# rg2/DeepFluoroLabeling-IPCAI2020

Hardware: AMD Instinct MI355X
Metric: train images/sec, paper U-Net (depth 6, wf 5, BN, strided-conv down, seg + 14-landmark heads), 1x192x192 (8x-downsampled 184x184 padded) (higher is better)
Workload: dtype bf16 (bf16 activations, activation gradients and GEMM weight copies in HBM; bf16 MFMA, fp32 accumulate, BatchNorm statistics, losses, weight gradients and master weights); 1 GPU; BASELINE configs[1]: 8x-downsampled, seg + 14-landmark heat-map dual head, batch 16 per GPU, Dice+NCC loss, SGD nesterov; global_batch=16, image=1x192x192, parallelism=dp1, math=bf16s, optimizer=dfl_amd.SGD(momentum 0.9, nesterov, wd 1e-4)

## Files before the change

deepfluorolabeling-ipcai2020_amd/csrc/convp.h:

```cpp
#pragma once
#include "common.h"

namespace dfl {

struct ConvP {
  dfl_conv_args a;
  int Mtot, Cout;
  int Hg, Wg;
  int PH, PW, IPP;
  int npy, npx, npatch;
  int IH, IW;
  int CK, nblk, blk_per_slice;
  int splits, T;
  int pix_stride, upp_shift;
  int lds_bytes, tile;
  int ntiles, grid, xcd_mode;
  uint32_t x_bytes, w_bytes;
  uint32_t x2_bytes, xo_bytes;
  uint32_t mPP, mPW;
  int tab_off, pad1;
  int s_mt, s_nt, s_ksplit_shift, s_cpk_shift, s_ksteps, s_kper;
  uint32_t qm_npatch, qm_ntiles, qm_perimg, qm_npx;
  int q_ngroups, q_stride;
};
constexpr int CONVS_TILE = 39;
constexpr int CONVQ_TILE = 40;
constexpr int CONVQ_LAYOUTS = 9;
constexpr int CONVN_TILE = 58;
constexpr int CONVN_LAYOUTS = 6;
constexpr int CONVN_PERS_TILE = 64;

int convp_plan(const dfl_conv_args* a, ConvP* p, int force_splits);
int convp_launch(const ConvP& p, hipStream_t s);
int convp_finish_rows(const ConvP& p);
int convp_candidates(const dfl_conv_args* a, int32_t* out, int max);
int convp_force(const int32_t* g);
int convp_tune_add(const int32_t* key, const int32_t* g);

bool convq_shape_ok(const dfl_conv_args& a);
int convq_launch(const ConvP& p, int mode, int pers, hipStream_t s);
size_t convq_lds_bytes(int ck, int mode, int blk_per_slice, int pers);
int convq_threads(int mode);
bool convq_pers_ok(int mode, int ck, int x_mode);
bool convq_ck_ok(int mode, int ck);

bool convn_shape_ok(const dfl_conv_args& a);
bool convn_layout_ok(int layout, int ntot, int cin);
void convn_patch(int layout, int* ph, int* pw);
size_t convn_lds_bytes(int layout, int cin, int ntot, int pers);
bool convn_pers_ok(int layout, const dfl_conv_args& a);
int convn_launch(const ConvP& p, int layout, int pers, hipStream_t s);

bool convs_eligible(const dfl_conv_args& a, const ConvP& p);
void convs_plan(const dfl_conv_args& a, ConvP* p, int force_splits);
int convs_launch(const ConvP& p, hipStream_t s);
bool convs_first_ok(const dfl_conv_args* a);
int convs_first_launch(const dfl_conv_args* a, hipStream_t s);
int convs_pair_ok(const dfl_conv_args* a, const dfl_conv_args* b);
int convs_pair_launch(const dfl_conv_args* a, const dfl_conv_args* b, hipStream_t s);

bool convs32_eligible(const dfl_conv_args* a);
int convs32_suggest_splits(const dfl_conv_args* a);
int convs32_launch(const dfl_conv_args* a, hipStream_t s, int* splits_out);
int convs32_pair_ok(const dfl_conv_args* a, const dfl_conv_args* b);
int convs32_pair_launch(const dfl_conv_args* a, const dfl_conv_args* b, hipStream_t s);

struct WgP;
int wgradp_suggest_splits(const dfl_wgrad_args* a);
int wgradp_launch(const dfl_wgrad_args* a, hipStream_t s);
int wgradp_config(const dfl_wgrad_args* a);

}
```

deepfluorolabeling-ipcai2020_amd/csrc/wgradp_bf16.hip:

```cpp
#include <stdlib.h>
#include <string.h>

#include <mutex>
#include <vector>

#include "common.h"
#include "convp.h"

namespace dfl {

constexpr uint32_t WPOOB = 0x80000000u;
typedef unsigned int wpu32x4 __attribute__((ext_vector_type(4)));
typedef short ws16x4_t __attribute__((ext_vector_type(4)));

struct WgP {
  dfl_wgrad_args a;
  int Mtot, T;
  int PH, PW, IPP, npy, npx, npatch;
  int IH, IW;
  int P16;
  int CMT, CGT;
  int pairs, phases;
  int zslices, patches_per_slice;
  int sd, sg;
  int dupp_shift, gupp_shift;
  int g_off;
  int tab_off;
  int lds_bytes;
  long long* trace;
  uint32_t g_bytes, d_bytes;
  uint32_t d2_bytes;
  int xcd_map;
};

__device__ __forceinline__ float wbf_lo(uint32_t w) { return __uint_as_float(w << 16); }
__device__ __forceinline__ float wbf_hi(uint32_t w) { return __uint_as_float(w & 0xffff0000u); }
__device__ __forceinline__ uint32_t wpack_bf2(float a, float b) {
  const bf16x2_t h = __builtin_convertvector((f32x2_t){a, b}, bf16x2_t);
  return __builtin_bit_cast(uint32_t, h);
}

__device__ __forceinline__ bf16x8_t wtr_read8(const unsigned char* base, uint32_t r0, uint32_t r1) {
  typedef __attribute__((address_space(3))) ws16x4_t* lds_p;
  const ws16x4_t x = __builtin_amdgcn_ds_read_tr16_b64_v4i16((lds_p)(base + r0));
  const ws16x4_t y = __builtin_amdgcn_ds_read_tr16_b64_v4i16((lds_p)(base + r1));
  return __builtin_bit_cast(bf16x8_t, __builtin_shufflevector(x, y, 0, 1, 2, 3, 4, 5, 6, 7));
}

typedef unsigned int wpu32x2 __attribute__((ext_vector_type(2)));
__device__ __forceinline__ wpu32x2 wtr_read4(const unsigned char* base, uint32_t r0) {
  typedef __attribute__((address_space(3))) ws16x4_t* lds_p;
  return __builtin_bit_cast(wpu32x2, __builtin_amdgcn_ds_read_tr16_b64_v4i16((lds_p)(base + r0)));
}

__host__ __device__ constexpr int wgp_max_d_units(int KH, bool dbrb = false) { return KH == 3 ? (dbrb ? 1536 : 2304) : 1024; }
__host__ __device__ constexpr int wgp_max_g_units(int KH, bool dbrb = false) { return KH == 3 ? (dbrb ? 3072 : 4608) : 2048; }

template <int KH, int KW, bool AFF, bool DBRB = false, bool BIAS = DBRB>
__global__ void __launch_bounds__(256 * KH, KH == 2 ? 4 : 3) wgradp_kernel(const WgP p) {
  constexpr int NT = 256 * KH;
  constexpr int T = KH * KW;
  extern __shared__ __attribute__((aligned(16))) unsigned char smem[];
  const dfl_wgrad_args& a = p.a;
#ifdef DFL_WGP_TRACE
  const long long tr_entry = __builtin_amdgcn_s_memtime();
#endif
  const int tid = threadIdx.x, lane = tid & 63, wave = tid >> 6;
  const int li = lane & 31, lh = lane >> 5;
  const int ty = wave % KH, slot = wave / KH;
  const int pair = slot % p.pairs, phase = slot / p.pairs;
  const int pairs_n = p.CGT >> 5;
  const int pm = pair / pairs_n, pn = pair - pm * pairs_n;
  int bx = blockIdx.x, by = blockIdx.y, bz = blockIdx.z;
  if (p.xcd_map) {
    const int gx = gridDim.x, gy = gridDim.y, nt = gx * gy;
    const int total = nt * (int)gridDim.z, per = total >> 3;
    const int L = bx + gx * (by + gy * bz);
    const int Lp = L < (per << 3) ? (L & 7) * per + (L >> 3) : L;
    bz = Lp / nt;
    const int t = Lp - bz * nt;
    bx = t / gy;
    by = t - bx * gy;
  }
  const int cm0 = bx * p.CMT, cg0 = by * p.CGT;
  unsigned char* Ds = smem;
  unsigned char* Gs = smem + p.g_off;

  __amdgpu_buffer_rsrc_t rsD = __builtin_amdgcn_make_buffer_rsrc(const_cast<float*>(a.d), 0, (int)p.d_bytes, 0x00020000);
  __amdgpu_buffer_rsrc_t rsG = __builtin_amdgcn_make_buffer_rsrc(const_cast<float*>(a.g), 0, (int)p.g_bytes, 0x00020000);
  __amdgpu_buffer_rsrc_t rsD2 = rsD;
  if constexpr (DBRB) rsD2 = __builtin_amdgcn_make_buffer_rsrc(const_cast<float*>(a.d2), 0, (int)p.d2_bytes, 0x00020000);

  f32x16 acc[KW];
#pragma unroll
  for (int t = 0; t < KW; ++t)
#pragma unroll
    for (int r = 0; r < 16; ++r) acc[t][r] = 0.f;

  const int trow = 8 * lh + ((lane & 15) >> 2);
  const uint32_t tcb = (uint32_t)((16 * ((lane >> 4) & 1) + 4 * (lane & 3)) * 2);
  const uint32_t d_col = (uint32_t)(pm * 64) + tcb, g_col = (uint32_t)(pn * 64) + tcb;

  const int dupp = p.CMT >> 3, gupp = p.CGT >> 3;
  const int npix_g = p.IPP * p.IH * p.IW;
  const int per_img = p.npy * p.npx;
  uint32_t* gtab = reinterpret_cast<uint32_t*>(smem + p.tab_off);

  constexpr int MAXD = wgp_max_d_units(KH, DBRB) / NT, MAXG = wgp_max_g_units(KH, DBRB) / NT;
  wpu32x4 dreg[MAXD], greg[MAXG];
  wpu32x4 d2reg[DBRB ? MAXD : 1];
  float bsum = 0.f;
  const bool bias_on = BIAS && a.bias_partial != nullptr && by == 0;
  uint32_t dpos[MAXD], gpos[MAXG];
  uint32_t gok = 0;
  const int ddk = NT >> p.dupp_shift, gdk = NT >> p.gupp_shift;
  const int dcq = tid & (dupp - 1), gcq = tid & (gupp - 1);
  const int dc = cm0 + dcq * 8, gc = cg0 + gcq * 8;
  const uint32_t dpitch = (uint32_t)a.ldd * 2u, gpitch = (uint32_t)a.ldg * 2u, d2pitch = (uint32_t)a.ldd2 * 2u;
  const int nd = (p.P16 * dupp + NT - 1) / NT, ng = (npix_g * gupp + NT - 1) / NT;
  {
    const int PHW = p.PH * p.PW;
#pragma unroll
    for (int u = 0; u < MAXD; ++u) {
      const int k = (tid >> p.dupp_shift) + u * ddk;
      const int img = k / PHW, r = k - img * PHW;
      const int y = r / p.PW, x = r - y * p.PW;
      const bool live = k < p.P16 && img < p.IPP && dc < a.Cm;
      dpos[u] = (uint32_t)y | ((uint32_t)x << 12) | ((uint32_t)(img & 127) << 24) | (live ? 0x80000000u : 0u);
    }
    const int IHW = p.IH * p.IW;
#pragma unroll
    for (int u = 0; u < MAXG; ++u) {
      const int k = (tid >> p.gupp_shift) + u * gdk;
      const int img = k / IHW, r = k - img * IHW;
      const int y = r / p.IW, x = r - y * p.IW;
      const bool live = k < npix_g && gc < a.Cg;
      gpos[u] = (uint32_t)y | ((uint32_t)x << 12) | ((uint32_t)(img & 127) << 24) | (live ? 0x80000000u : 0u);
    }
    for (int j = tid; j < p.P16; j += NT) {
      const int img = j / PHW, r = j - img * PHW;
      const int y = r / p.PW, x = r - y * p.PW;
      gtab[j] = img < p.IPP ? (uint32_t)((img * p.IH + y * a.stride) * p.IW + x * a.stride) * (uint32_t)p.sg : 0u;
    }
  }
  float* aff = reinterpret_cast<float*>(smem + p.tab_off + p.P16 * 4);
  float* dco = aff + 2 * p.CGT;
  int is_nleft = 0, is_oy0 = 0, is_ox0 = 0, is_ybase = 0, is_xbase = 0;
  uint32_t is_dbase = 0, is_dbase2 = 0, is_gbase = 0;
  auto issue_setup = [&](int patch, bool live) {
    const int pg = patch / per_img, pr = patch - pg * per_img;
    const int ppy = pr / p.npx, ppx = pr - ppy * p.npx;
    const int img0 = pg * p.IPP;
    is_oy0 = ppy * p.PH;
    is_ox0 = ppx * p.PW;
    is_nleft = live ? a.N - img0 : 0;
    is_dbase = (uint32_t)(((img0 * a.Hout + is_oy0) * a.Wout + is_ox0) * a.ldd + dc) * 2u;
    is_dbase2 = DBRB ? (uint32_t)(((img0 * a.Hout + is_oy0) * a.Wout + is_ox0) * a.ldd2 + dc) * 2u : 0u;
    is_ybase = is_oy0 * a.stride - a.pad;
    is_xbase = is_ox0 * a.stride - a.pad;
    is_gbase = (uint32_t)(((img0 * a.Hin + is_ybase) * a.Win + is_xbase) * a.ldg + gc) * 2u;
    gok = 0;
  };
  auto issue_d = [&](int u) {
    if (u < nd) {
      const uint32_t q = dpos[u];
      const int qy = (int)(q & 0xfffu), qx = (int)((q >> 12) & 0xfffu), qi = (int)((q >> 24) & 127u);
      const bool ok = (int)q < 0 && qi < is_nleft && is_oy0 + qy < a.Hout && is_ox0 + qx < a.Wout;
      const uint32_t rel = (uint32_t)((qi * a.Hout + qy) * a.Wout + qx) * dpitch;
      dreg[u] = __builtin_amdgcn_raw_buffer_load_b128(rsD, ok ? is_dbase + rel : WPOOB, 0, 0);
      if constexpr (DBRB) {
        const uint32_t rel2 = (uint32_t)((qi * a.Hout + qy) * a.Wout + qx) * d2pitch;
        d2reg[u] = __builtin_amdgcn_raw_buffer_load_b128(rsD2, ok ? is_dbase2 + rel2 : WPOOB, 0, 0);
      }
    }
  };
  auto issue_g = [&](int u) {
    if (u < ng) {
      const uint32_t q = gpos[u];
      const int qy = (int)(q & 0xfffu), qx = (int)((q >> 12) & 0xfffu), qi = (int)((q >> 24) & 127u);
      const bool ok = (int)q < 0 && qi < is_nleft && (unsigned)(is_ybase + qy) < (unsigned)a.Hin && (unsigned)(is_xbase + qx) < (unsigned)a.Win;
      gok |= ok ? (1u << u) : 0u;
      const uint32_t rel = (uint32_t)((qi * a.Hin + qy) * a.Win + qx) * gpitch;
      greg[u] = __builtin_amdgcn_raw_buffer_load_b128(rsG, ok ? is_gbase + rel : WPOOB, 0, 0);
    }
  };
  auto issue = [&](int patch, bool live) {
    issue_setup(patch, live);
#pragma unroll
    for (int u = 0; u < MAXD; ++u) issue_d(u);
#pragma unroll
    for (int u = 0; u < MAXG; ++u) issue_g(u);
  };
  auto commit = [&]() {
#pragma unroll
    for (int u = 0; u < MAXD; ++u) {
      const int k = (tid >> p.dupp_shift) + u * ddk;
      if (u < nd && k < p.P16) {
        wpu32x4 v = dreg[u];
        if constexpr (DBRB) {
          const wpu32x4 r = d2reg[u];
          const float4 a0 = *reinterpret_cast<const float4*>(dco + dcq * 8), a1 = *reinterpret_cast<const float4*>(dco + dcq * 8 + 4);
          const float4 b0 = *reinterpret_cast<const float4*>(dco + p.CMT + dcq * 8), b1 = *reinterpret_cast<const float4*>(dco + p.CMT + dcq * 8 + 4);
          const float4 c0 = *reinterpret_cast<const float4*>(dco + 2 * p.CMT + dcq * 8), c1 = *reinterpret_cast<const float4*>(dco + 2 * p.CMT + dcq * 8 + 4);
          auto brb = [](float dy, float rv, float A, float B, float Cc) { return rv > 0.f ? fmaf(A, dy, fmaf(B, rv, Cc)) : 0.f; };
          v.x = wpack_bf2(brb(wbf_lo(v.x), wbf_lo(r.x), a0.x, b0.x, c0.x), brb(wbf_hi(v.x), wbf_hi(r.x), a0.y, b0.y, c0.y));
          v.y = wpack_bf2(brb(wbf_lo(v.y), wbf_lo(r.y), a0.z, b0.z, c0.z), brb(wbf_hi(v.y), wbf_hi(r.y), a0.w, b0.w, c0.w));
          v.z = wpack_bf2(brb(wbf_lo(v.z), wbf_lo(r.z), a1.x, b1.x, c1.x), brb(wbf_hi(v.z), wbf_hi(r.z), a1.y, b1.y, c1.y));
          v.w = wpack_bf2(brb(wbf_lo(v.w), wbf_lo(r.w), a1.z, b1.z, c1.z), brb(wbf_hi(v.w), wbf_hi(r.w), a1.w, b1.w, c1.w));
        }
        *reinterpret_cast<wpu32x4*>(Ds + (uint32_t)k * (uint32_t)p.sd + (uint32_t)dcq * 16u) = v;
      }
    }
#pragma unroll
    for (int u = 0; u < MAXG; ++u) {
      const int pix = (tid >> p.gupp_shift) + u * gdk;
      if (u < ng && pix < npix_g) {
        wpu32x4 v = greg[u];
        if constexpr (AFF) {
          if ((gok >> u) & 1u) {
            const float4 s0 = *reinterpret_cast<const float4*>(aff + gcq * 8), s1 = *reinterpret_cast<const float4*>(aff + gcq * 8 + 4);
            const float4 h0 = *reinterpret_cast<const float4*>(aff + p.CGT + gcq * 8), h1 = *reinterpret_cast<const float4*>(aff + p.CGT + gcq * 8 + 4);
            const float sc[8] = {s0.x, s0.y, s0.z, s0.w, s1.x, s1.y, s1.z, s1.w}, sh[8] = {h0.x, h0.y, h0.z, h0.w, h1.x, h1.y, h1.z, h1.w};
            v.x = wpack_bf2(fmaf(wbf_lo(v.x), sc[0], sh[0]), fmaf(wbf_hi(v.x), sc[1], sh[1]));
            v.y = wpack_bf2(fmaf(wbf_lo(v.y), sc[2], sh[2]), fmaf(wbf_hi(v.y), sc[3], sh[3]));
            v.z = wpack_bf2(fmaf(wbf_lo(v.z), sc[4], sh[4]), fmaf(wbf_hi(v.z), sc[5], sh[5]));
            v.w = wpack_bf2(fmaf(wbf_lo(v.w), sc[6], sh[6]), fmaf(wbf_hi(v.w), sc[7], sh[7]));
          }
        }
        *reinterpret_cast<wpu32x4*>(Gs + (uint32_t)pix * (uint32_t)p.sg + (uint32_t)gcq * 16u) = v;
      }
    }
  };

  const int pbegin = bz * p.patches_per_slice;
  const int pend = min(pbegin + p.patches_per_slice, p.npatch);
  const int nsteps = p.P16 >> 4;
  const uint32_t gadd = g_col + (uint32_t)(ty * p.IW) * (uint32_t)p.sg;
  const uint32_t dstep = (uint32_t)(16 * p.phases) * (uint32_t)p.sd;
  const bool al8 = KW == 3 && a.stride == 1 && (p.PW & 7) == 0;
#ifdef DFL_WGP_TRACE
  long long tr[8] = {0, 0, 0, 0, 0, 0, 0, 0};
  tr[0] = __builtin_amdgcn_s_memtime();
  tr[6] = __builtin_amdgcn_s_memrealtime();
#define WTR(i, t0) tr[i] += __builtin_amdgcn_s_memtime() - (t0);
#define WT0(name) const long long name = __builtin_amdgcn_s_memtime();
#else
#define WTR(i, t0)
#define WT0(name)
#endif
  issue(pbegin, pbegin < pend);
  if constexpr (AFF) {
    for (int c = tid; c < p.CGT; c += NT) {
      aff[c] = (cg0 + c < a.Cg) ? a.in_scale[cg0 + c] : 1.f;
      aff[p.CGT + c] = (cg0 + c < a.Cg) ? a.in_shift[cg0 + c] : 0.f;
    }
  }
  if constexpr (DBRB) {
    for (int c = tid; c < p.CMT; c += NT) {
      const bool live = a.coef != nullptr && cm0 + c < a.Cm;
      float A = live ? a.coef[cm0 + c] : 1.f, B = live ? a.coef[a.Cm + cm0 + c] : 0.f, Cc = live ? a.coef[2 * a.Cm + cm0 + c] : 0.f;
      if (a.coef_tot != nullptr && cm0 + c < a.Cm)
        bn_live_coef(a.coef_tot, a.bn_gamma, a.bn_mean, a.bn_invstd, a.bn_count, a.Cm, cm0 + c, &A, &B, &Cc);
      dco[c] = A;
      dco[p.CMT + c] = B;
      dco[2 * p.CMT + c] = Cc;
    }
  }
  if constexpr (AFF || DBRB) __syncthreads();
  for (int patch = pbegin; patch < pend; ++patch) {
    WT0(tb0)
    if (patch != pbegin) __syncthreads();
    WTR(1, tb0)
    WT0(tc0)
    commit();
    WTR(2, tc0)
    WT0(tb1)
    __syncthreads();
    WTR(1, tb1)
    WT0(ti0)
    issue(patch + 1, patch + 1 < pend);
    WTR(3, ti0)
    if constexpr (BIAS) {
      if (bias_on) {
        const int bc = tid & (p.CMT - 1), bstride = NT / p.CMT;
        for (int r = tid / p.CMT; r < p.P16; r += bstride)
          bsum += __uint_as_float((uint32_t)*reinterpret_cast<const unsigned short*>(Ds + (uint32_t)r * (uint32_t)p.sd + (uint32_t)bc * 2u) << 16);
      }
    }
    WT0(tk0)
    uint32_t dr0 = (uint32_t)(phase * 16 + trow) * (uint32_t)p.sd + d_col;
    const uint32_t* tp = gtab + phase * 16 + trow;
    int ks = phase;
    auto kstep = [&]() {
      const uint32_t gr0 = tp[0] + gadd, gr1 = tp[4] + gadd;
      const bf16x8_t df = wtr_read8(Ds, dr0, dr0 + 4u * (uint32_t)p.sd);
      bf16x8_t gf[KW];
      if (KW == 3 && al8) {
        const wpu32x2 g0 = wtr_read4(Gs, gr0), g1 = wtr_read4(Gs, gr1), g2 = wtr_read4(Gs, gr0 + 8u * (uint32_t)p.sg);
        gf[0] = __builtin_bit_cast(bf16x8_t, (wpu32x4){g0.x, g0.y, g1.x, g1.y});
        gf[1] = __builtin_bit_cast(bf16x8_t, (wpu32x4){__builtin_amdgcn_alignbit(g0.y, g0.x, 16), __builtin_amdgcn_alignbit(g1.x, g0.y, 16),
                                                        __builtin_amdgcn_alignbit(g1.y, g1.x, 16), __builtin_amdgcn_alignbit(g2.x, g1.y, 16)});
        gf[KW - 1] = __builtin_bit_cast(bf16x8_t, (wpu32x4){g0.y, g1.x, g1.y, g2.x});
      } else {
#pragma unroll
        for (int t = 0; t < KW; ++t) gf[t] = wtr_read8(Gs, gr0 + (uint32_t)(t * p.sg), gr1 + (uint32_t)(t * p.sg));
      }
#pragma unroll
      for (int t = 0; t < KW; ++t) acc[t] = __builtin_amdgcn_mfma_f32_32x32x16_bf16(df, gf[t], acc[t], 0, 0, 0);
      dr0 += dstep;
      tp += 16 * p.phases;
      ks += p.phases;
    };
    while (ks < nsteps) kstep();
    WTR(4, tk0)
  }
#ifdef DFL_WGP_TRACE
  tr[5] = __builtin_amdgcn_s_memtime();
#endif

  if constexpr (BIAS) {
    if (a.bias_partial != nullptr && by == 0) {
      __syncthreads();
      float* bred = reinterpret_cast<float*>(smem);
      bred[tid] = bsum;
      __syncthreads();
      for (int c = tid; c < p.CMT; c += NT) {
        float t = 0.f;
        for (int th = c; th < NT; th += p.CMT) t += bred[th];
        if (cm0 + c < a.Cm) a.bias_partial[(int64_t)bz * a.Cm + cm0 + c] = t;
      }
    }
  }

  if (p.phases > 1) {
    float* red = reinterpret_cast<float*>(smem);
#pragma unroll
    for (int t = 0; t < KW; ++t) {
      __syncthreads();
      if (phase > 0) {
        float* dst = red + ((((phase - 1) * p.pairs + pair) * KH + ty) * 16) * 64 + lane;
#pragma unroll
        for (int r = 0; r < 16; ++r) dst[r * 64] = acc[t][r];
      }
      __syncthreads();
      if (phase == 0) {
        for (int ph = 1; ph < p.phases; ++ph) {
          const float* src = red + ((((ph - 1) * p.pairs + pair) * KH + ty) * 16) * 64 + lane;
#pragma unroll
          for (int r = 0; r < 16; ++r) acc[t][r] += src[r * 64];
        }
      }
    }
    if (phase > 0 && p.zslices > 1) return;
  }
#ifdef DFL_WGP_TRACE
  const long long tr_main_end = __builtin_amdgcn_s_memtime();
#endif
  const bool sliced = p.zslices > 1;
  const int cgl = pn * 32 + li, cg = cg0 + cgl;
  if (sliced) {
    float* out = a.partial + (int64_t)bz * a.Cm * a.Cg * T;
#pragma unroll
    for (int tx = 0; tx < KW; ++tx) {
      const int t = ty * KW + tx;
#pragma unroll
      for (int r = 0; r < 16; ++r) {
        const int cm = cm0 + pm * 32 + mfma32_row(r, lane);
        if (cm < a.Cm && cg < a.Cg) out[((int64_t)t * a.Cm + cm) * a.Cg + cg] = acc[tx][r];
      }
    }
  } else {
    __syncthreads();
    float* tile = reinterpret_cast<float*>(smem);
    if (phase == 0) {
#pragma unroll
      for (int tx = 0; tx < KW; ++tx) {
        const int t = ty * KW + tx;
#pragma unroll
        for (int r = 0; r < 16; ++r) tile[((pm * 32 + mfma32_row(r, lane)) * p.CGT + cgl) * T + t] = acc[tx][r];
      }
    }
    __syncthreads();
    const int row4 = p.CGT * T / 4;
    const int valid4 = min(p.CGT, a.Cg - cg0) * T / 4;
    for (int idx = tid; idx < p.CMT * row4; idx += NT) {
      const int row = idx / row4, c4 = idx - row * row4;
      if (cm0 + row < a.Cm && c4 < valid4)
        *reinterpret_cast<float4*>(a.dw + ((int64_t)(cm0 + row) * a.Cg + cg0) * T + c4 * 4) = *reinterpret_cast<const float4*>(tile + (row * p.CGT) * T + c4 * 4);
    }
  }
#ifdef DFL_WGP_TRACE
  __builtin_amdgcn_s_waitcnt(0);
  if (tid == 0 && p.trace != nullptr) {
    long long* sink = p.trace + (int64_t)(blockIdx.x + gridDim.x * (blockIdx.y + gridDim.y * blockIdx.z)) * 12;
    for (int i = 0; i < 6; ++i) sink[i] = tr[i];
    sink[6] = tr_main_end;
    sink[7] = tr[6];
    sink[8] = __builtin_amdgcn_s_memrealtime();
    sink[10] = tr_entry;
    sink[11] = __builtin_amdgcn_s_memtime();
    sink[9] = 1;
  }
#endif
}


static int pitch_for(int channels) {
  const int data = channels * 2;
  int pitch = data;
  while (pitch % 256 != 64 && pitch % 256 != 192) pitch += 16;
  return pitch;
}

static int wgp_plan(const dfl_wgrad_args* a, WgP* p, bool need_out) {
  DFL_REQUIRE(a != nullptr, "dfl_conv2d_wgrad: null args");
  DFL_REQUIRE(a->N > 0 && a->Hin > 0 && a->Win > 0 && a->Cg > 0 && a->Cm > 0, "dfl_conv2d_wgrad: bad sizes");
  DFL_REQUIRE(a->KH > 0 && a->KW > 0 && a->stride > 0 && a->pad >= 0, "dfl_conv2d_wgrad: bad window");
  const int T = a->KH * a->KW;
  DFL_REQUIRE((a->KH == 1 && a->KW == 1) || (a->KH == 2 && a->KW == 2) || (a->KH == 3 && a->KW == 3),
              "dfl_conv2d_wgrad (bf16): 1x1, 2x2 and 3x3 windows");
  const int ho = (a->Hin + 2 * a->pad - a->KH) / a->stride + 1;
  const int wo = (a->Win + 2 * a->pad - a->KW) / a->stride + 1;
  DFL_REQUIRE(ho == a->Hout && wo == a->Wout, "dfl_conv2d_wgrad: Hout/Wout (%d,%d) do not match the window (%d,%d)", a->Hout,
              a->Wout, ho, wo);
  DFL_REQUIRE(a->Cg % 8 == 0 && a->Cm % 8 == 0 && a->ldg % 8 == 0 && a->ldd % 8 == 0 && aligned16(a->g) && aligned16(a->d),
              "dfl_conv2d_wgrad (bf16): channel counts and pixel strides must be multiples of 8, tensors 16-byte aligned");
  DFL_REQUIRE((a->in_scale == nullptr) == (a->in_shift == nullptr), "dfl_conv2d_wgrad: in_scale/in_shift go together");
  if (need_out) {
    DFL_REQUIRE(a->g && a->d, "dfl_conv2d_wgrad: g and d are required");
    DFL_REQUIRE(a->splits >= 1, "dfl_conv2d_wgrad: splits >= 1");
    DFL_REQUIRE(a->splits > 1 ? a->partial != nullptr : a->dw != nullptr, "dfl_conv2d_wgrad: output buffer missing");
  }
  memset(p, 0, sizeof(*p));
  p->a = *a;
  p->T = T;
  const int64_t M = (int64_t)a->N * a->Hout * a->Wout;
  DFL_REQUIRE(M < (1ll << 31), "dfl_conv2d_wgrad: too many pixels");
  p->Mtot = (int)M;
  const int64_t gb = (((int64_t)a->N * a->Hin * a->Win - 1) * a->ldg + a->Cg) * 2;
  const int64_t db = ((M - 1) * a->ldd + a->Cm) * 2;
  const int64_t lim = (1ll << 31) - 4096;
  DFL_REQUIRE(gb < lim && db < lim, "dfl_conv2d_wgrad (bf16): tensors must stay below 2 GiB");
  p->g_bytes = (uint32_t)gb;
  p->d_bytes = (uint32_t)db;
  if (a->d_mode != 0) {
    DFL_REQUIRE(a->coef_tot == nullptr || (a->coef == nullptr && a->bn_gamma && a->bn_mean && a->bn_invstd && a->bn_count > 0),
                "dfl_conv2d_wgrad (bf16): coef_tot replaces coef and needs bn_gamma, bn_mean, bn_invstd, bn_count");
    DFL_REQUIRE(a->d_mode == 1 && a->KH == 3 && a->d2 != nullptr && a->ldd2 % 8 == 0 && aligned16(a->d2),
                "dfl_conv2d_wgrad (bf16): d_mode 1 needs a 3x3 window and d2 (16-byte aligned, ldd2 %% 8 == 0)");
    const int64_t d2b = ((M - 1) * a->ldd2 + a->Cm) * 2;
    DFL_REQUIRE(d2b < lim, "dfl_conv2d_wgrad (bf16): tensors must stay below 2 GiB");
    p->d2_bytes = (uint32_t)d2b;
  }
  DFL_REQUIRE(a->bias_partial == nullptr || a->KH == 3, "dfl_conv2d_wgrad (bf16): bias_partial is implemented by the 3x3 kernel");
  p->CMT = a->Cm > 32 ? 64 : 32;
  p->CGT = a->Cg > 32 ? 64 : 32;
  {
    static const int small_from = [] {
      const char* e = getenv("DFL_WGP_SMALL_TILES");
      return e ? atoi(e) : 4;
    }();
    constexpr int small_from21 = 4;
    const int64_t tiles64 = ceil_div(a->Cm, 64) * ceil_div(a->Cg, 64);
    const int from = a->KH == 3 ? small_from : small_from21;
    if (from > 0 && a->Cm > 32 && a->Cg > 32 && tiles64 >= from && tiles64 < 256) p->CMT = p->CGT = 32;
  }
  p->pairs = (p->CMT / 32) * (p->CGT / 32);
  p->phases = 4 / p->pairs;
  p->dupp_shift = p->CMT == 64 ? 3 : 2;
  p->gupp_shift = p->CGT == 64 ? 3 : 2;
  p->sd = pitch_for(p->CMT);
  p->sg = pitch_for(p->CGT);
  const int64_t max_du = wgp_max_d_units(a->KH, a->d_mode != 0), max_gu = wgp_max_g_units(a->KH, a->d_mode != 0);
  const int lds_cap = a->KH == 3 ? 120 * 1024 : (a->KH == 2 ? 72 * 1024 : 52 * 1024);
  auto geom = [&](int ipp_, int ph_, int pw_, int64_t* lds, int64_t* du, int64_t* gu) {
    const int p16 = (ipp_ * ph_ * pw_ + 15) / 16 * 16;
    const int ih = (ph_ - 1) * a->stride + a->KH, iw = (pw_ - 1) * a->stride + a->KW;
    *du = (int64_t)p16 * (p->CMT / 8);
    *gu = (int64_t)ipp_ * ih * iw * (p->CGT / 8);
    *lds = (int64_t)p16 * p->sd + (int64_t)ipp_ * ih * iw * p->sg + (int64_t)p16 * 4 + 512;
  };
  auto fits = [&](int ipp_, int ph_, int pw_) {
    int64_t lds, du, gu;
    geom(ipp_, ph_, pw_, &lds, &du, &gu);
    return lds <= lds_cap && du <= max_du && gu <= max_gu && ipp_ <= 127 && ph_ < 4096 && pw_ < 4096;
  };
  int ipp = 0, ph = 0, pw = 0;
  double best_cost = 1e300;
  struct PatchMemo { int key[8]; int ipp, ph, pw; };
  static std::mutex memo_mu;
  static std::vector<PatchMemo> memo;
  const int mkey[8] = {a->N, a->Hout, a->Wout, a->stride, a->KH + 16 * (a->d_mode != 0 ? 1 : 0), a->KW, p->CMT, p->CGT};
  bool found = false;
  {
    std::lock_guard<std::mutex> lock(memo_mu);
    for (const PatchMemo& m : memo)
      if (memcmp(m.key, mkey, sizeof(mkey)) == 0) {
        ipp = m.ipp; ph = m.ph; pw = m.pw;
        found = true;
        break;
      }
  }
  auto consider = [&](int ipp_, int ph_, int pw_) {
    if (ipp_ < 1 || ph_ < 1 || pw_ < 1 || ph_ > a->Hout || pw_ > a->Wout || !fits(ipp_, ph_, pw_)) return;
    int64_t lds, du, gu;
    geom(ipp_, ph_, pw_, &lds, &du, &gu);
    const double npatch = (double)ceil_div(a->N, ipp_) * (double)ceil_div(a->Hout, ph_) * (double)ceil_div(a->Wout, pw_);
    constexpr double charge = 24.0 * 1024.0;
    double cost = npatch * ((double)(du + gu) * 16.0 + charge);
    if (a->KH == 3 && a->stride == 1 && pw_ % 8 == 0) cost *= 0.92;
    if (cost < best_cost) {
      best_cost = cost;
      ipp = ipp_;
      ph = ph_;
      pw = pw_;
    }
  };
  if (!found) {
    for (int n = a->N; n >= 1; --n) consider(n, a->Hout, a->Wout);
    for (int pw_ = 4; pw_ <= a->Wout; ++pw_) {
      if (pw_ != a->Wout && pw_ % 4 != 0) continue;
      for (int ph_ = 1; ph_ <= a->Hout; ++ph_) {
        if (!fits(1, ph_, pw_)) break;
        consider(1, ph_, pw_);
      }
    }
    if (ipp == 0) consider(1, 1, a->Wout < 4 ? a->Wout : 4);
    DFL_REQUIRE(ipp > 0, "dfl_conv2d_wgrad (bf16): no patch of this layer fits the staging limits");
    PatchMemo m;
    memcpy(m.key, mkey, sizeof(mkey));
    m.ipp = ipp; m.ph = ph; m.pw = pw;
    std::lock_guard<std::mutex> lock(memo_mu);
    if (memo.size() < 4096) memo.push_back(m);
  }
  p->IPP = ipp;
  p->PH = ph;
  p->PW = pw;
  p->P16 = (ipp * ph * pw + 15) / 16 * 16;
  p->npy = (int)ceil_div(a->Hout, ph);
  p->npx = (int)ceil_div(a->Wout, pw);
  p->npatch = (int)ceil_div(a->N, ipp) * p->npy * p->npx;
  p->IH = (ph - 1) * a->stride + a->KH;
  p->IW = (pw - 1) * a->stride + a->KW;
  p->g_off = (p->P16 * p->sd + 255) / 256 * 256;
  p->tab_off = (p->g_off + (ipp * p->IH * p->IW + 2) * p->sg + 255) / 256 * 256;
  p->lds_bytes = p->tab_off + p->P16 * 4 + 2 * p->CGT * 4 + 3 * p->CMT * 4;
  if ((a->d_mode != 0 || a->bias_partial != nullptr) && p->lds_bytes < 256 * a->KH * 4) p->lds_bytes = 256 * a->KH * 4;
  const int red_bytes = (p->phases - 1) * p->pairs * a->KH * 16 * 64 * 4;
  if (p->lds_bytes < red_bytes) p->lds_bytes = red_bytes;
  return DFL_OK;
}

static int wgp_slices(const WgP& p) {
  const int64_t tiles = ceil_div(p.a.Cm, p.CMT) * ceil_div(p.a.Cg, p.CGT);
  constexpr int target3 = 256;
  constexpr int target21 = 512;
  const int target = p.a.KH == 3 ? target3 : target21;
  int64_t z = ceil_div(target, tiles);
  if (z > p.npatch) z = p.npatch;
  if (z < 1) z = 1;
  const int64_t pps = ceil_div(p.npatch, z);
  z = ceil_div(p.npatch, pps);
  return (int)z;
}

int wgradp_suggest_splits(const dfl_wgrad_args* a) {
  WgP p;
  int rc = wgp_plan(a, &p, false);
  if (rc != DFL_OK) return rc;
  return wgp_slices(p);
}

int wgradp_config(const dfl_wgrad_args* a) {
  WgP p;
  int rc = wgp_plan(a, &p, false);
  if (rc != DFL_OK) return rc;
  return 16 + (p.T == 9 ? 0 : (p.T == 4 ? 1 : 2));
}

template <int KH, int KW>
static int wgp_launch_t(const WgP& p_in, hipStream_t s) {
  WgP p = p_in;
  dim3 grid((unsigned)ceil_div(p.a.Cm, p.CMT), (unsigned)ceil_div(p.a.Cg, p.CGT), (unsigned)p.zslices);
  p.xcd_map = (grid.x * grid.y > 1 && grid.x * grid.y * grid.z >= 16) ? 1 : 0;
  const size_t lds = (size_t)p.lds_bytes;
#define DFL_WGP_LAUNCH(AFF_, DBRB_, BIAS_)                                                                                       \
  {                                                                                                                              \
    auto k = wgradp_kernel<KH, KW, AFF_, DBRB_, BIAS_>;                                                                          \
    DFL_LDS_OPT_IN(k, 150 * 1024, "dfl_conv2d_wgrad (bf16)") \
    hipLaunchKernelGGL(k, grid, dim3(256 * KH), lds, s, p);                                                                      \
  }
  const bool aff = p.a.in_scale != nullptr;
  if constexpr (KH == 3) {
    if (p.a.d_mode != 0) {
      if (aff) DFL_WGP_LAUNCH(true, true, true) else DFL_WGP_LAUNCH(false, true, true)
      return check_launch("dfl_conv2d_wgrad (bf16)");
    }
    if (p.a.bias_partial != nullptr) {
      if (aff) DFL_WGP_LAUNCH(true, false, true) else DFL_WGP_LAUNCH(false, false, true)
      return check_launch("dfl_conv2d_wgrad (bf16)");
    }
  }
  if (aff) DFL_WGP_LAUNCH(true, false, false) else DFL_WGP_LAUNCH(false, false, false)
#undef DFL_WGP_LAUNCH
  return check_launch("dfl_conv2d_wgrad (bf16)");
}

int wgradp_launch(const dfl_wgrad_args* a, hipStream_t s) {
  WgP p;
  int rc = wgp_plan(a, &p, true);
  if (rc != DFL_OK) return rc;
  p.zslices = a->splits;
  p.patches_per_slice = (int)ceil_div(p.npatch, p.zslices);
  if (p.zslices == 1 && p.lds_bytes < p.CMT * p.CGT * p.T * 4) p.lds_bytes = p.CMT * p.CGT * p.T * 4;
#ifdef DFL_WGP_TRACE
  {
    const char* e = getenv("DFL_WGP_TRACE_PTR");
    p.trace = e ? reinterpret_cast<long long*>(strtoull(e, nullptr, 0)) : nullptr;
    fprintf(stderr, "wgradp: tile %dx%d pairs %d phases %d patch %dx%dx%d (P16 %d) gathered %dx%d slices %d patches/slice %d lds %d\n", p.CMT, p.CGT, p.pairs,
            p.phases, p.IPP, p.PH, p.PW, p.P16, p.IH, p.IW, p.zslices, p.patches_per_slice, p.lds_bytes);
  }
#endif
  switch (p.T) {
    case 9: return wgp_launch_t<3, 3>(p, s);
    case 4: return wgp_launch_t<2, 2>(p, s);
    default: return wgp_launch_t<1, 1>(p, s);
  }
}

}
```

Measured before the change: 4523 images/sec.

## Add row-streaming 3x3 weight-gradient kernel with rolling input-row ring in LDS

```diff
diff --git a/deepfluorolabeling-ipcai2020_amd/csrc/convp.h b/deepfluorolabeling-ipcai2020_amd/csrc/convp.h
--- a/deepfluorolabeling-ipcai2020_amd/csrc/convp.h
+++ b/deepfluorolabeling-ipcai2020_amd/csrc/convp.h
@@ -69,5 +69,8 @@
 int wgradp_suggest_splits(const dfl_wgrad_args* a);
 int wgradp_launch(const dfl_wgrad_args* a, hipStream_t s);
 int wgradp_config(const dfl_wgrad_args* a);
+bool wgradn_applies(const dfl_wgrad_args* a);
+int wgradn_suggest_splits(const dfl_wgrad_args* a);
+int wgradn_launch(const dfl_wgrad_args* a, hipStream_t s);
 
 }
diff --git a/deepfluorolabeling-ipcai2020_amd/csrc/wgradn_bf16.hip b/deepfluorolabeling-ipcai2020_amd/csrc/wgradn_bf16.hip
--- /dev/null
+++ b/deepfluorolabeling-ipcai2020_amd/csrc/wgradn_bf16.hip
@@ -0,0 +1,448 @@
+#include <stdlib.h>
+#include <string.h>
+
+#include <algorithm>
+
+#include "common.h"
+#include "convp.h"
+
+namespace dfl {
+
+namespace {
+
+constexpr uint32_t WNOOB = 0x80000000u;
+constexpr int WN_NT = 512;
+typedef unsigned int wnu32x4 __attribute__((ext_vector_type(4)));
+typedef unsigned int wnu32x2 __attribute__((ext_vector_type(2)));
+typedef short wns16x4_t __attribute__((ext_vector_type(4)));
+
+template <bool DBRB> struct WnUnits { static constexpr int D = DBRB ? 2 : 3, G = 4; };
+
+struct WgN {
+  dfl_wgrad_args a;
+  int Hg;
+  int Vtot;
+  int PH, W16, GW, RG;
+  int CMT, CGT, pairs, phases;
+  int ncg, nb, RB;
+  int zslices, rows_per_slice;
+  int sd, sg;
+  int g_off, tab_off, lds_bytes;
+  uint32_t g_bytes, d_bytes, d2_bytes;
+};
+
+__device__ __forceinline__ float wn_lo(uint32_t w) { return __uint_as_float(w << 16); }
+__device__ __forceinline__ float wn_hi(uint32_t w) { return __uint_as_float(w & 0xffff0000u); }
+__device__ __forceinline__ uint32_t wn_pack(float a, float b) {
+  const bf16x2_t h = __builtin_convertvector((f32x2_t){a, b}, bf16x2_t);
+  return __builtin_bit_cast(uint32_t, h);
+}
+__device__ __forceinline__ wnu32x2 wn_tr4(const unsigned char* base, uint32_t off) {
+  typedef __attribute__((address_space(3))) wns16x4_t* lds_p;
+  return __builtin_bit_cast(wnu32x2, __builtin_amdgcn_ds_read_tr16_b64_v4i16((lds_p)(base + off)));
+}
+
+template <bool AFF, bool DBRB, bool BIAS>
+__global__ void __launch_bounds__(WN_NT, 2) wgradn_kernel(const WgN p) {
+  constexpr int NT = WN_NT;
+  constexpr int MAXD = WnUnits<DBRB>::D, MAXG = WnUnits<DBRB>::G;
+  extern __shared__ __attribute__((aligned(16))) unsigned char smem[];
+  const dfl_wgrad_args& a = p.a;
+  const int tid = threadIdx.x, lane = tid & 63, wave = tid >> 6;
+  const int pair = wave % p.pairs, phase = wave / p.pairs;
+  const int pairs_n = p.CGT >> 5;
+  const int pm = pair / pairs_n, pn = pair - pm * pairs_n;
+  const int bz = blockIdx.z;
+  const int cm0 = blockIdx.x * p.CMT, cg0 = blockIdx.y * p.CGT;
+  unsigned char* Ds = smem;
+  unsigned char* Gs = smem + p.g_off;
+  float* aff = reinterpret_cast<float*>(smem + p.tab_off);
+  float* dco = aff + 2 * p.CGT;
+
+  __amdgpu_buffer_rsrc_t rsD = __builtin_amdgcn_make_buffer_rsrc(const_cast<float*>(a.d), 0, (int)p.d_bytes, 0x00020000);
+  __amdgpu_buffer_rsrc_t rsG = __builtin_amdgcn_make_buffer_rsrc(const_cast<float*>(a.g), 0, (int)p.g_bytes, 0x00020000);
+  __amdgpu_buffer_rsrc_t rsD2 = rsD;
+  if constexpr (DBRB) rsD2 = __builtin_amdgcn_make_buffer_rsrc(const_cast<float*>(a.d2), 0, (int)p.d2_bytes, 0x00020000);
+
+  const int dupp = p.CMT >> 3, gupp = p.CGT >> 3;
+  const int dcq = tid & (dupp - 1), gcq = tid & (gupp - 1);
+  const int dk0 = tid / dupp, dks = NT / dupp, gk0 = tid / gupp, gks = NT / gupp;
+  const int dc = cm0 + dcq * 8, gc = cg0 + gcq * 8;
+  const int dpix = p.PH * p.W16, gpix = p.PH * p.GW;
+  const uint32_t dpitch = (uint32_t)a.ldd * 2u, gpitch = (uint32_t)a.ldg * 2u, d2pitch = (uint32_t)a.ldd2 * 2u;
+  uint32_t dpos[MAXD], gpos[MAXG];
+#pragma unroll
+  for (int u = 0; u < MAXD; ++u) {
+    const int k = dk0 + u * dks, y = k / p.W16, x = k - y * p.W16;
+    dpos[u] = (k < dpix && x < a.Wout && dc < a.Cm) ? ((uint32_t)y | ((uint32_t)x << 16)) : 0xffffffffu;
+  }
+#pragma unroll
+  for (int u = 0; u < MAXG; ++u) {
+    const int k = gk0 + u * gks, y = k / p.GW, x = k - y * p.GW;
+    const int ix = x - a.pad;
+    gpos[u] = (k < gpix && ix >= 0 && ix < a.Win && gc < a.Cg) ? ((uint32_t)y | ((uint32_t)x << 16)) : 0xffffffffu;
+  }
+  wnu32x4 dreg[MAXD], greg[MAXG];
+  wnu32x4 d2reg[DBRB ? MAXD : 1];
+  uint32_t gok = 0;
+  int is_gslot = 0;
+
+  const int v0 = bz * p.rows_per_slice;
+  const int v1 = min(v0 + p.rows_per_slice, p.Vtot);
+  auto issue = [&](int pi) {
+    const int vb = v0 + pi * p.PH;
+    if (pi >= 0) {
+      const int img0 = vb / p.Hg, oy0 = vb - img0 * p.Hg;
+#pragma unroll
+      for (int u = 0; u < MAXD; ++u) {
+        const uint32_t q = dpos[u];
+        const int y = (int)(q & 0xffffu), x = (int)(q >> 16);
+        int oy = oy0 + y, img = img0;
+        if (oy >= p.Hg) { oy -= p.Hg; ++img; }
+        const bool ok = q != 0xffffffffu && vb + y < v1 && oy < a.Hout && img < a.N;
+        const uint32_t row = (uint32_t)(img * a.Hout + oy) * (uint32_t)a.Wout + (uint32_t)x;
+        dreg[u] = __builtin_amdgcn_raw_buffer_load_b128(rsD, ok ? row * dpitch + (uint32_t)dc * 2u : WNOOB, 0, 0);
+        if constexpr (DBRB) d2reg[u] = __builtin_amdgcn_raw_buffer_load_b128(rsD2, ok ? row * d2pitch + (uint32_t)dc * 2u : WNOOB, 0, 0);
+      }
+    }
+    const int Y0 = vb + 2;
+    const int Yc = Y0 < 0 ? 0 : Y0;
+    const int img0 = Yc / p.Hg, y0 = Yc - img0 * p.Hg;
+    is_gslot = ((Y0 % p.RG) + p.RG) % p.RG;
+    gok = 0;
+#pragma unroll
+    for (int u = 0; u < MAXG; ++u) {
+      const uint32_t q = gpos[u];
+      const int y = (int)(q & 0xffffu), x = (int)(q >> 16);
+      int yy = y0 + y + (Y0 < 0 ? Y0 : 0), img = img0;
+      if (yy >= p.Hg) { yy -= p.Hg; ++img; }
+      const int iy = yy - a.pad;
+      const bool ok = q != 0xffffffffu && Y0 + y >= 0 && iy >= 0 && iy < a.Hin && img < a.N;
+      gok |= ok ? (1u << u) : 0u;
+      const uint32_t pix = (uint32_t)(img * a.Hin + iy) * (uint32_t)a.Win + (uint32_t)(x - a.pad);
+      greg[u] = __builtin_amdgcn_raw_buffer_load_b128(rsG, ok ? pix * gpitch + (uint32_t)gc * 2u : WNOOB, 0, 0);
+    }
+  };
+  auto commit = [&](bool with_d) {
+    if (with_d) {
+#pragma unroll
+      for (int u = 0; u < MAXD; ++u) {
+        const int k = dk0 + u * dks;
+        if (k < dpix) {
+          wnu32x4 v = dreg[u];
+          if constexpr (DBRB) {
+            const wnu32x4 r = d2reg[u];
+            const float4 a0 = *reinterpret_cast<const float4*>(dco + dcq * 8), a1 = *reinterpret_cast<const float4*>(dco + dcq * 8 + 4);
+            const float4 b0 = *reinterpret_cast<const float4*>(dco + p.CMT + dcq * 8), b1 = *reinterpret_cast<const float4*>(dco + p.CMT + dcq * 8 + 4);
+            const float4 c0 = *reinterpret_cast<const float4*>(dco + 2 * p.CMT + dcq * 8), c1 = *reinterpret_cast<const float4*>(dco + 2 * p.CMT + dcq * 8 + 4);
+            auto brb = [](float dy, float rv, float A, float B, float Cc) { return rv > 0.f ? fmaf(A, dy, fmaf(B, rv, Cc)) : 0.f; };
+            v.x = wn_pack(brb(wn_lo(v.x), wn_lo(r.x), a0.x, b0.x, c0.x), brb(wn_hi(v.x), wn_hi(r.x), a0.y, b0.y, c0.y));
+            v.y = wn_pack(brb(wn_lo(v.y), wn_lo(r.y), a0.z, b0.z, c0.z), brb(wn_hi(v.y), wn_hi(r.y), a0.w, b0.w, c0.w));
+            v.z = wn_pack(brb(wn_lo(v.z), wn_lo(r.z), a1.x, b1.x, c1.x), brb(wn_hi(v.z), wn_hi(r.z), a1.y, b1.y, c1.y));
+            v.w = wn_pack(brb(wn_lo(v.w), wn_lo(r.w), a1.z, b1.z, c1.z), brb(wn_hi(v.w), wn_hi(r.w), a1.w, b1.w, c1.w));
+          }
+          *reinterpret_cast<wnu32x4*>(Ds + (uint32_t)k * (uint32_t)p.sd + (uint32_t)dcq * 16u) = v;
+        }
+      }
+    }
+#pragma unroll
+    for (int u = 0; u < MAXG; ++u) {
+      const int k = gk0 + u * gks;
+      if (k < gpix) {
+        const int y = k / p.GW, x = k - y * p.GW;
+        int slot = is_gslot + y;
+        if (slot >= p.RG) slot -= p.RG;
+        wnu32x4 v = greg[u];
+        if constexpr (AFF) {
+          if ((gok >> u) & 1u) {
+            const float4 s0 = *reinterpret_cast<const float4*>(aff + gcq * 8), s1 = *reinterpret_cast<const float4*>(aff + gcq * 8 + 4);
+            const float4 h0 = *reinterpret_cast<const float4*>(aff + p.CGT + gcq * 8), h1 = *reinterpret_cast<const float4*>(aff + p.CGT + gcq * 8 + 4);
+            v.x = wn_pack(fmaf(wn_lo(v.x), s0.x, h0.x), fmaf(wn_hi(v.x), s0.y, h0.y));
+            v.y = wn_pack(fmaf(wn_lo(v.y), s0.z, h0.z), fmaf(wn_hi(v.y), s0.w, h0.w));
+            v.z = wn_pack(fmaf(wn_lo(v.z), s1.x, h1.x), fmaf(wn_hi(v.z), s1.y, h1.y));
+            v.w = wn_pack(fmaf(wn_lo(v.w), s1.z, h1.z), fmaf(wn_hi(v.w), s1.w, h1.w));
+          }
+        }
+        *reinterpret_cast<wnu32x4*>(Gs + (uint32_t)(slot * p.GW + x) * (uint32_t)p.sg + (uint32_t)gcq * 16u) = v;
+      }
+    }
+  };
+
+  f32x16 acc[9];
+#pragma unroll
+  for (int t = 0; t < 9; ++t)
+#pragma unroll
+    for (int r = 0; r < 16; ++r) acc[t][r] = 0.f;
+  float bsum = 0.f;
+  const bool bias_on = BIAS && a.bias_partial != nullptr && blockIdx.y == 0;
+
+  const int npatch = v1 > v0 ? (v1 - v0 + p.PH - 1) / p.PH : 0;
+  const int npro = p.PH >= 2 ? 1 : 2;
+  issue(-npro);
+  if constexpr (AFF) {
+    for (int c = tid; c < p.CGT; c += NT) {
+      aff[c] = (cg0 + c < a.Cg) ? a.in_scale[cg0 + c] : 1.f;
+      aff[p.CGT + c] = (cg0 + c < a.Cg) ? a.in_shift[cg0 + c] : 0.f;
+    }
+  }
+  if constexpr (DBRB) {
+    for (int c = tid; c < p.CMT; c += NT) {
+      const bool live = a.coef != nullptr && cm0 + c < a.Cm;
+      float A = live ? a.coef[cm0 + c] : 1.f, B = live ? a.coef[a.Cm + cm0 + c] : 0.f, Cc = live ? a.coef[2 * a.Cm + cm0 + c] : 0.f;
+      if (a.coef_tot != nullptr && cm0 + c < a.Cm)
+        bn_live_coef(a.coef_tot, a.bn_gamma, a.bn_mean, a.bn_invstd, a.bn_count, a.Cm, cm0 + c, &A, &B, &Cc);
+      dco[c] = A;
+      dco[p.CMT + c] = B;
+      dco[2 * p.CMT + c] = Cc;
+    }
+  }
+  if constexpr (AFF || DBRB) __syncthreads();
+  commit(false);
+  if (npro == 2) {
+    issue(-1);
+    commit(false);
+  }
+  if (npatch > 0) issue(0);
+
+  const int lh = lane >> 5, q = (lane & 15) >> 2;
+  const uint32_t tcb = (uint32_t)((16 * ((lane >> 4) & 1) + 4 * (lane & 3)) * 2);
+  const uint32_t d_col = (uint32_t)(pm * 64) + tcb, g_col = (uint32_t)(pn * 64) + tcb;
+  const uint32_t sd = (uint32_t)p.sd, sg = (uint32_t)p.sg;
+  const int nitems = p.ncg * p.nb;
+
+  for (int pi = 0; pi < npatch; ++pi) {
+    __syncthreads();
+    commit(true);
+    __syncthreads();
+    const int vb = v0 + pi * p.PH;
+    if (pi + 1 < npatch) issue(pi + 1);
+    if constexpr (BIAS) {
+      if (bias_on) {
+        const int bc = tid & (p.CMT - 1), bstride = NT / p.CMT;
+        for (int r = tid / p.CMT; r < dpix; r += bstride)
+          bsum += __uint_as_float((uint32_t)*reinterpret_cast<const unsigned short*>(Ds + (uint32_t)r * sd + (uint32_t)bc * 2u) << 16);
+      }
+    }
+    const int rows = min(p.PH, v1 - vb);
+    const int sbase = vb % p.RG;
+    for (int it = phase; it < nitems; it += p.phases) {
+      const int cgi = it % p.ncg, band = it / p.ncg;
+      const int r0 = band * p.RB, r1 = min(rows, r0 + p.RB);
+      if (r0 >= r1) continue;
+      const uint32_t xoff = (uint32_t)(cgi * 16 + 8 * lh + q);
+      const unsigned char* dbase = Ds + xoff * sd + d_col;
+      const unsigned char* gbase = Gs + xoff * sg + g_col;
+      auto gload = [&](int r, wnu32x2& x0, wnu32x2& x1, wnu32x2& x2) {
+        int s = sbase + r;
+        if (s >= p.RG) s -= p.RG;
+        if (s >= p.RG) s -= p.RG;
+        const uint32_t o = (uint32_t)(s * p.GW) * sg;
+        x0 = wn_tr4(gbase, o);
+        x1 = wn_tr4(gbase, o + 4u * sg);
+        x2 = wn_tr4(gbase, o + 8u * sg);
+      };
+      wnu32x2 a0, a1, a2, b0, b1, b2;
+      gload(r0, a0, a1, a2);
+      gload(r0 + 1, b0, b1, b2);
+      for (int r = r0; r < r1; ++r) {
+        wnu32x2 c0, c1, c2;
+        gload(r + 2, c0, c1, c2);
+        const uint32_t od = (uint32_t)(r * p.W16) * sd;
+        const wnu32x2 e0 = wn_tr4(dbase, od), e1 = wn_tr4(dbase, od + 4u * sd);
+        const bf16x8_t df = __builtin_bit_cast(bf16x8_t, (wnu32x4){e0.x, e0.y, e1.x, e1.y});
+        auto taps = [&](int ky, const wnu32x2& g0, const wnu32x2& g1, const wnu32x2& g2) {
+          const bf16x8_t f0 = __builtin_bit_cast(bf16x8_t, (wnu32x4){g0.x, g0.y, g1.x, g1.y});
+          const bf16x8_t f1 = __builtin_bit_cast(bf16x8_t, (wnu32x4){__builtin_amdgcn_alignbit(g0.y, g0.x, 16), __builtin_amdgcn_alignbit(g1.x, g0.y, 16),
+                                                                      __builtin_amdgcn_alignbit(g1.y, g1.x, 16), __builtin_amdgcn_alignbit(g2.x, g1.y, 16)});
+          const bf16x8_t f2 = __builtin_bit_cast(bf16x8_t, (wnu32x4){g0.y, g1.x, g1.y, g2.x});
+          acc[ky * 3 + 0] = __builtin_amdgcn_mfma_f32_32x32x16_bf16(df, f0, acc[ky * 3 + 0], 0, 0, 0);
+          acc[ky * 3 + 1] = __builtin_amdgcn_mfma_f32_32x32x16_bf16(df, f1, acc[ky * 3 + 1], 0, 0, 0);
+          acc[ky * 3 + 2] = __builtin_amdgcn_mfma_f32_32x32x16_bf16(df, f2, acc[ky * 3 + 2], 0, 0, 0);
+        };
+        taps(0, a0, a1, a2);
+        taps(1, b0, b1, b2);
+        taps(2, c0, c1, c2);
+        a0 = b0; a1 = b1; a2 = b2;
+        b0 = c0; b1 = c1; b2 = c2;
+      }
+    }
+  }
+
+  if constexpr (BIAS) {
+    if (bias_on) {
+      __syncthreads();
+      float* bred = reinterpret_cast<float*>(smem);
+      bred[tid] = bsum;
+      __syncthreads();
+      for (int c = tid; c < p.CMT; c += NT) {
+        float t = 0.f;
+        for (int th = c; th < NT; th += p.CMT) t += bred[th];
+        if (cm0 + c < a.Cm) a.bias_partial[(int64_t)bz * a.Cm + cm0 + c] = t;
+      }
+    }
+  }
+  if (p.phases > 1) {
+    float* red = reinterpret_cast<float*>(smem);
+#pragma unroll
+    for (int t = 0; t < 9; ++t) {
+      __syncthreads();
+      if (phase > 0) {
+        float* dst = red + (((phase - 1) * p.pairs + pair) * 16) * 64 + lane;
+#pragma unroll
+        for (int r = 0; r < 16; ++r) dst[r * 64] = acc[t][r];
+      }
+      __syncthreads();
+      if (phase == 0) {
+        for (int ph = 1; ph < p.phases; ++ph) {
+          const float* src = red + (((ph - 1) * p.pairs + pair) * 16) * 64 + lane;
+#pragma unroll
+          for (int r = 0; r < 16; ++r) acc[t][r] += src[r * 64];
+        }
+      }
+    }
+    if (phase > 0) return;
+  }
+  const int cg = cg0 + pn * 32 + (lane & 31);
+  if (p.zslices > 1) {
+    float* out = a.partial + (int64_t)bz * a.Cm * a.Cg * 9;
+#pragma unroll
+    for (int t = 0; t < 9; ++t)
+#pragma unroll
+      for (int r = 0; r < 16; ++r) {
+        const int cm = cm0 + pm * 32 + mfma32_row(r, lane);
+        if (cm < a.Cm && cg < a.Cg) out[((int64_t)t * a.Cm + cm) * a.Cg + cg] = acc[t][r];
+      }
+  } else {
+#pragma unroll
+    for (int r = 0; r < 16; ++r) {
+      const int cm = cm0 + pm * 32 + mfma32_row(r, lane);
+      if (cm < a.Cm && cg < a.Cg) {
+        float* o = a.dw + ((int64_t)cm * a.Cg + cg) * 9;
+#pragma unroll
+        for (int t = 0; t < 9; ++t) o[t] = acc[t][r];
+      }
+    }
+  }
+}
+
+int wn_pitch(int channels) {
+  int pitch = channels * 2;
+  while (pitch % 256 != 64 && pitch % 256 != 192) pitch += 16;
+  return pitch;
+}
+
+bool wn_enabled() {
+  static const bool on = [] {
+    const char* e = getenv("DFL_WGRADN");
+    return !(e && e[0] == '0');
+  }();
+  return on;
+}
+
+}
+
+bool wgradn_applies(const dfl_wgrad_args* a) {
+  if (!wn_enabled() || a == nullptr) return false;
+  if (!(a->g_bf16 && a->d_bf16 && a->KH == 3 && a->KW == 3 && a->stride == 1 && (a->pad == 0 || a->pad == 1))) return false;
+  if (a->Cg % 32 != 0 || a->Cm % 32 != 0 || a->Wout < 24 || a->Hout < 1) return false;
+  if (a->d_split != 0) return false;
+  return true;
+}
+
+static int wn_plan(const dfl_wgrad_args* a, WgN* p) {
+  memset(p, 0, sizeof(*p));
+  p->a = *a;
+  DFL_REQUIRE(a->Hout + 2 == a->Hin + 2 * a->pad && a->Wout + 2 == a->Win + 2 * a->pad, "dfl_conv2d_wgrad (wgradn): 3x3 stride-1 geometry");
+  p->Hg = a->Hout + 2;
+  const int64_t vt = (int64_t)a->N * p->Hg;
+  DFL_REQUIRE(vt < (1ll << 30), "dfl_conv2d_wgrad (wgradn): too many rows");
+  p->Vtot = (int)vt;
+  const int64_t M = (int64_t)a->N * a->Hout * a->Wout;
+  const int64_t gb = (((int64_t)a->N * a->Hin * a->Win - 1) * a->ldg + a->Cg) * 2;
+  const int64_t db = ((M - 1) * a->ldd + a->Cm) * 2;
+  const int64_t lim = (1ll << 31) - 4096;
+  DFL_REQUIRE(gb < lim && db < lim, "dfl_conv2d_wgrad (bf16): tensors must stay below 2 GiB");
+  p->g_bytes = (uint32_t)gb;
+  p->d_bytes = (uint32_t)db;
+  if (a->d_mode != 0) {
+    const int64_t d2b = ((M - 1) * a->ldd2 + a->Cm) * 2;
+    DFL_REQUIRE(d2b < lim, "dfl_conv2d_wgrad (bf16): tensors must stay below 2 GiB");
+    p->d2_bytes = (uint32_t)d2b;
+  }
+  p->CMT = 32;
+  p->CGT = 32;
+  p->pairs = 1;
+  p->phases = 8;
+  p->sd = wn_pitch(p->CMT);
+  p->sg = wn_pitch(p->CGT);
+  p->W16 = (a->Wout + 15) / 16 * 16;
+  p->GW = p->W16 + 4;
+  p->ncg = p->W16 / 16;
+  const bool dbrb = a->d_mode != 0;
+  const int maxd = (dbrb ? WnUnits<true>::D : WnUnits<false>::D) * WN_NT, maxg = (dbrb ? WnUnits<true>::G : WnUnits<false>::G) * WN_NT;
+  const int dupr = p->W16 * (p->CMT / 8), gupr = p->GW * (p->CGT / 8);
+  int ph = std::min(maxd / dupr, maxg / gupr);
+  DFL_REQUIRE(ph >= 1, "dfl_conv2d_wgrad (wgradn): rows of %d pixels do not fit the staging budget", a->Wout);
+  if (ph > p->Hg) ph = p->Hg;
+  p->PH = ph;
+  p->RG = ph + 2;
+  int best_nb = 1;
+  double best = 1e300;
+  for (int nb = 1; nb <= ph; ++nb) {
+    const int rb = (ph + nb - 1) / nb;
+    const int items = p->ncg * nb;
+    const int per_wave = (items + p->phases - 1) / p->phases;
+    const double cost = (double)per_wave * (rb * 14.0 + 6.0);
+    if (cost < best - 1e-9) { best = cost; best_nb = nb; }
+  }
+  p->nb = best_nb;
+  p->RB = (ph + best_nb - 1) / best_nb;
+  p->g_off = (ph * p->W16 * p->sd + 255) / 256 * 256;
+  p->tab_off = (p->g_off + p->RG * p->GW * p->sg + 255) / 256 * 256;
+  p->lds_bytes = p->tab_off + 2 * p->CGT * 4 + 3 * p->CMT * 4;
+  const int red = (p->phases - 1) * p->pairs * 16 * 64 * 4;
+  if (p->lds_bytes < red) p->lds_bytes = red;
+  if (p->lds_bytes < WN_NT * 4) p->lds_bytes = WN_NT * 4;
+  return DFL_OK;
+}
+
+int wgradn_suggest_splits(const dfl_wgrad_args* a) {
+  WgN p;
+  const int rc = wn_plan(a, &p);
+  if (rc != DFL_OK) return rc;
+  const int64_t tiles = ceil_div(a->Cm, p.CMT) * ceil_div(a->Cg, p.CGT);
+  const int64_t npatch = ceil_div(p.Vtot, p.PH);
+  int64_t z = ceil_div(256, tiles);
+  if (z > npatch) z = npatch;
+  if (z < 1) z = 1;
+  const int64_t pps = ceil_div(npatch, z);
+  return (int)ceil_div(npatch, pps);
+}
+
+int wgradn_launch(const dfl_wgrad_args* a, hipStream_t s) {
+  WgN p;
+  const int rc = wn_plan(a, &p);
+  if (rc != DFL_OK) return rc;
+  p.zslices = a->splits;
+  p.rows_per_slice = (int)(ceil_div(ceil_div(p.Vtot, p.PH), p.zslices) * p.PH);
+  dim3 grid((unsigned)ceil_div(a->Cm, p.CMT), (unsigned)ceil_div(a->Cg, p.CGT), (unsigned)p.zslices);
+  const size_t lds = (size_t)p.lds_bytes;
+#define DFL_WGN_LAUNCH(AFF_, DBRB_, BIAS_)                                          \
+  {                                                                                 \
+    auto k = wgradn_kernel<AFF_, DBRB_, BIAS_>;                                     \
+    DFL_LDS_OPT_IN(k, 150 * 1024, "dfl_conv2d_wgrad (wgradn)")                      \
+    hipLaunchKernelGGL(k, grid, dim3(WN_NT), lds, s, p);                            \
+  }
+  const bool aff = a->in_scale != nullptr;
+  if (a->d_mode != 0) {
+    if (aff) DFL_WGN_LAUNCH(true, true, true) else DFL_WGN_LAUNCH(false, true, true)
+  } else if (a->bias_partial != nullptr) {
+    if (aff) DFL_WGN_LAUNCH(true, false, true) else DFL_WGN_LAUNCH(false, false, true)
+  } else {
+    if (aff) DFL_WGN_LAUNCH(true, false, false) else DFL_WGN_LAUNCH(false, false, false)
+  }
+#undef DFL_WGN_LAUNCH
+  return check_launch("dfl_conv2d_wgrad (wgradn)");
+}
+
+}
diff --git a/deepfluorolabeling-ipcai2020_amd/csrc/wgradp_bf16.hip b/deepfluorolabeling-ipcai2020_amd/csrc/wgradp_bf16.hip
--- a/deepfluorolabeling-ipcai2020_amd/csrc/wgradp_bf16.hip
+++ b/deepfluorolabeling-ipcai2020_amd/csrc/wgradp_bf16.hip
@@ -568,6 +568,7 @@
   WgP p;
   int rc = wgp_plan(a, &p, false);
   if (rc != DFL_OK) return rc;
+  if (wgradn_applies(a)) return wgradn_suggest_splits(a);
   return wgp_slices(p);
 }
 
@@ -610,6 +611,7 @@
   WgP p;
   int rc = wgp_plan(a, &p, true);
   if (rc != DFL_OK) return rc;
+  if (wgradn_applies(a)) return wgradn_launch(a, s);
   p.zslices = a->splits;
   p.patches_per_slice = (int)ceil_div(p.npatch, p.zslices);
   if (p.zslices == 1 && p.lds_bytes < p.CMT * p.CGT * p.T * 4) p.lds_bytes = p.CMT * p.CGT * p.T * 4;
```

Result: slower. 4193 images/sec (median of 2 runs) (-7.3%).
